# gorgonia/agogo

Measured on AMD Instinct MI355X. Metric: mcts_sims_per_sec, higher is better.
Workload: dtype f32 (Winograd F(5x5,3x3): fp32 transforms; transform-domain products as fp16x2 = each fp32 operand scaled by a power of two and split into 2 fp16 pieces (22-23 significand bits, absolute error <= 2^-38 of the tensor range), 3 fp16 MFMAs per product, fp32 accumulate)

## Files before the change

### agogo_amd/capi.py

```python
import ctypes as C
import os

import numpy as np

_HERE = os.path.dirname(os.path.abspath(__file__))
_LIB = None

NONE, BLACK, WHITE = 0, 1, 2
PASS, RESIGN = -1, -2
NO_MOVE = -32768
GAME_MNK, GAME_C4, GAME_KOMI, GAME_WQ = 0, 1, 2, 3
ENC_TWOPLANE, ENC_WQ = 0, 1
INF_NET, INF_DUMMY, INF_SCRIPT, INF_HASH, INF_UNIFORM, INF_CALLBACK = 0, 1, 2, 3, 4, 5
BN_DEGENERATE_EPS, BN_RUNNING, BN_IDENTITY = 0, 1, 2
COMPUTE_F32_MFMA, COMPUTE_BF16X3, COMPUTE_FP16X2, COMPUTE_WINO, COMPUTE_AUTO, COMPUTE_WINO_H2 = 0, 1, 2, 3, 4, 5
COMPUTE_FORCE = 0x100
PROF_CONV, PROF_HEADS, PROF_SELECT, PROF_EXPAND, PROF_MOVE, PROF_CONV_INIT = 0, 1, 2, 3, 4, 5
PROF_WINO_IN, PROF_WINO_GEMM, PROF_WINO_OUT = 6, 7, 8
DONT_PREFER_PASS, PREFER_PASS, DONT_RESIGN = 0, 1, 2
POOL_STRICT, POOL_STOP_SEARCH, POOL_GROW = 0, 1, 2


class AgzError(RuntimeError):
    pass
# ... 190 lines not shown
    sig("agz_arena_examples_dev", i32, vp, pvp, pvp, pvp, pi)
    i64, pi64 = C.c_int64, C.POINTER(C.c_int64)
    sig("agz_train_dev", i32, vp, vp, vp, vp, i32, i32, u64, pf)
    sig("agz_examples_create", i32, vp, i32, i32, i32, i32, pvp)
    sig("agz_examples_destroy", None, vp)
    sig("agz_examples_count", i32, vp, pi64)
    sig("agz_examples_clear", i32, vp)
    sig("agz_examples_append_arena", i32, vp, vp)
    sig("agz_examples_append_dev", i32, vp, vp, vp, vp, i64)
    sig("agz_examples_append_host", i32, vp, pf, pf, pf, i64)
    sig("agz_examples_get", i32, vp, pf, pf, pf, i64, pi64)
    sig("agz_examples_augment_rotate", i32, vp)
    sig("agz_examples_prepare", i32, vp, i32, i32, u64, pi)
    sig("agz_examples_tensors_dev", i32, vp, pvp, pvp, pvp, pi64, pi)
    sig("agz_examples_get_tensors", i32, vp, pf, pf, pf)
    sig("agz_examples_raw_dev", i32, vp, pvp, pvp, pvp)
    sig("agz_rotate_boards", i32, vp, pf, i32, i32, i32, pf)
    sig("agz_ctx_prof_set_stride", i32, vp, i32, i32)
    sig("agz_wino_stages", i32, vp, pf, pf, i32, i32, i32, i32, i32, pf, pf)
    sig("agz_wino_h2_tile", i32, i32, i32)
    sig("agz_net_set_wino_h2_form", i32, vp, i32)
    sig("agz_net_set_wino_h2_gemm", i32, vp, i32)
    sig("agz_net_wino_h2_last_rows", i32, vp, C.POINTER(C.c_int), C.POINTER(C.c_int))
    sig("agz_net_min_same_batch", i32, vp, i32, i32, C.POINTER(C.c_int))
    sig("agz_arena_set_prep_compact", i32, vp, i32)
    sig("agz_arena_set_split", i32, vp, i32)
    sig("agz_arena_split_steps", i32, vp, C.POINTER(C.c_int64), C.POINTER(C.c_int64), C.POINTER(C.c_int))
    sig("agz_trainer_set_dma_forward", i32, vp, i32)
    sig("agz_arena_last_prep_batch", i32, vp, C.POINTER(C.c_int), C.POINTER(C.c_int))
    sig("agz_arena_debug_counter", i32, vp, i32, C.POINTER(C.c_int64))
    sig("agz_arena_pool_capacity", i32, vp, C.POINTER(C.c_int), C.POINTER(C.c_int))
    sig("agz_wino_h2_chained", i32, i32, i32, i32)
    sig("agz_arena_random_moves", i32, vp, pi, u64)
    sig("agz_arena_set_state", i32, vp, i32, C.POINTER(State))
    sig("agz_arena_examples_labelled_dev", i32, vp, pvp)
    sig("agz_mcts_create", i32, vp, C.POINTER(GameConf), C.POINTER(MctsConf), u64, i32, pvp)
    sig("agz_mcts_destroy", None, vp)
    sig("agz_mcts_set_inferencer", i32, vp, i32, vp)
    sig("agz_mcts_set_inferencer_callback", i32, vp, INFER_FN, vp, i32)
    sig("agz_arena_set_inferencer_callback", i32, vp, i32, INFER_FN, vp, i32)
    sig("agz_arena_set_pool_policy", i32, vp, i32)
    sig("agz_mcts_set_pool_policy", i32, vp, i32)
    sig("agz_mcts_set_parallel", i32, vp, i32)
    sig("agz_mcts_set_game", i32, vp, C.POINTER(State))
    sig("agz_mcts_search", i32, vp, i32, pi)
    sig("agz_mcts_policies", i32, vp, pf, i32)
# ... 163 lines not shown
        _check(lib().agz_net_infer(self.h, _pf(x), B, _pf(pol), _pf(val)), "agz_net_infer")
        return pol, val

    def set_compute_mode(self, mode):
        _check(lib().agz_net_set_compute_mode(self.h, int(mode)), "agz_net_set_compute_mode")

    def set_latency_mode(self, on=True):
        _check(lib().agz_net_set_latency_mode(self.h, int(on)), "agz_net_set_latency_mode")

    def set_tower_queues(self, queues):
        _check(lib().agz_net_set_tower_queues(self.h, int(queues)), "agz_net_set_tower_queues")

    def set_wino_h2_form(self, form):
        _check(lib().agz_net_set_wino_h2_form(self.h, int(form)), "agz_net_set_wino_h2_form")

    def set_wino_h2_gemm(self, variant):
        _check(lib().agz_net_set_wino_h2_gemm(self.h, int(variant)), "agz_net_set_wino_h2_gemm")

    def wino_h2_last_rows(self):
        r, c = C.c_int(0), C.c_int(0)
        _check(lib().agz_net_wino_h2_last_rows(self.h, C.byref(r), C.byref(c)), "agz_net_wino_h2_last_rows")
        return r.value, c.value

    def min_same_batch(self, n, G):
        b = C.c_int(0)
        _check(lib().agz_net_min_same_batch(self.h, int(n), int(G), C.byref(b)), "agz_net_min_same_batch")
        return b.value

    def infer_dev(self, planes_ptr, B, policy_ptr, value_ptr):
        _check(lib().agz_net_infer_dev(self.h, C.c_void_p(planes_ptr), B, C.c_void_p(policy_ptr),
                                       C.c_void_p(value_ptr)), "agz_net_infer_dev")

    def flops_per_eval(self):
        return lib().agz_net_flops_per_eval(self.h)

    def save(self, path):
        _check(lib().agz_net_save(self.h, os.fsencode(path)), "agz_net_save")

    def load(self, path):
        _check(lib().agz_net_load(self.h, os.fsencode(path)), "agz_net_load")


class Trainer:

    def __init__(self, ctx, K, SharedLayers, FC, Width, Height, Features, ActionSpace, BatchSize, bn_eps=1e-5, tied=False):
        self.ctx = ctx
# ... 691 lines not shown
```

### agogo_amd/csrc/conv_wino_h2.hpp

```cpp
#pragma once

template <int TM> struct WinoT;
template <> struct WinoT<4> {
  static constexpr int AL = 6, VSHIFT = 7;
  static constexpr float BT[6][6] = {{4, 0, -5, 0, 1, 0}, {0, -4, -4, 1, 1, 0}, {0, 4, -4, -1, 1, 0}, {0, -2, -1, 2, 1, 0}, {0, 2, -1, -2, 1, 0}, {0, 4, 0, -5, 0, 1}};
  static constexpr float AT[4][6] = {{1, 1, 1, 1, 1, 0}, {0, 1, -1, 2, -2, 0}, {0, 1, 1, 4, 4, 0}, {0, 1, -1, 8, -8, 1}};
  static constexpr double G[6][3] = {{1.0 / 4, 0, 0}, {-1.0 / 6, -1.0 / 6, -1.0 / 6}, {-1.0 / 6, 1.0 / 6, -1.0 / 6}, {1.0 / 24, 1.0 / 12, 1.0 / 6}, {1.0 / 24, -1.0 / 12, 1.0 / 6}, {0, 0, 1}};
};
template <> struct WinoT<5> {
  static constexpr int AL = 7, VSHIFT = 6;
  static constexpr float BT[7][7] = {{-0.5f, 0.25f, 2.5f, -1.25f, -2, 1, 0}, {0, 0.5f, 0.25f, -2.25f, -1, 1, 0}, {0, -0.5f, 0.75f, 1.75f, -3, 1, 0},
                                     {0, 1, 1.5f, -2, -1.5f, 1, 0},          {0, -1, 2.5f, 0, -2.5f, 1, 0},       {0, 0.25f, 0, -1.25f, 0, 1, 0},
                                     {0, -0.5f, 0.25f, 2.5f, -1.25f, -2, 1}};
  static constexpr float AT[5][7] = {{1, 1, 1, 1, 1, 1, 0}, {0, 1, -1, 0.5f, -0.5f, 2, 0}, {0, 1, 1, 0.25f, 0.25f, 4, 0}, {0, 1, -1, 0.125f, -0.125f, 8, 0},
                                     {0, 1, 1, 0.0625f, 0.0625f, 16, 1}};
  static constexpr double G[7][3] = {{-2, 0, 0}, {-2.0 / 3, -2.0 / 3, -2.0 / 3}, {-2.0 / 9, 2.0 / 9, -2.0 / 9}, {16.0 / 9, 8.0 / 9, 4.0 / 9}, {16.0 / 15, -8.0 / 15, 4.0 / 15},
                                     {2.0 / 45, 4.0 / 45, 8.0 / 45}, {0, 0, 1}};
};
template <int TM> __device__ __forceinline__ void wino_btv(const float* d, float* o);
template <int TM> __device__ __forceinline__ void wino_atv(const float* m, float* o);
template <> __device__ __forceinline__ void wino_btv<4>(const float* d, float* o) { wino_bt6(d, o); }
template <> __device__ __forceinline__ void wino_atv<4>(const float* m, float* o) { wino_at4(m, o); }
template <> __device__ __forceinline__ void wino_btv<5>(const float* d, float* o) {
  o[0] = -0.5f * d[0] + 0.25f * d[1] + 2.5f * d[2] - 1.25f * d[3] - 2.f * d[4] + d[5];
// ... 25 lines not shown
  const float* w_unscale_dev;
  int fuse_prev;
  int wm_per_board;
  unsigned* amax_self;
  int in_swap;
  const _Float16* U2;
  const unsigned* amax_in;
  unsigned* amax_out;
  float* wave_max;
  float w_unscale;
  const float* t_in;
  const float* col_unscale;
  const float* t_next;
  int cform;
  const _Float16* U2c;
  const float* amax_true;
  const float* wm_prev;
  float* wm_out;
  unsigned* amax_next;
  float g1, g0;
  int gemm_variant;
  int temporal_stores;
  int live_r, live_c;
  int row_pad;
};
__device__ __forceinline__ size_t h2_row(const WinoH2Args& h, int pos, int t) {
  return (size_t)(t >> h.rsh) * h.rA + (size_t)pos * h.rB + (size_t)(t & h.rmask);
}

__device__ __forceinline__ void wino_h2_scales(unsigned amax_bits, int shift, float* s, float* inv) {
  int e = (int)((amax_bits >> 23) & 0xffu);
  if (amax_bits == 0u) { *s = 1.f; *inv = 1.f; return; }
  e = e < 30 ? 30 : (e > 230 ? 230 : e);
  *s = __uint_as_float((unsigned)(268 - shift - e) << 23);
  *inv = __uint_as_float((unsigned)(e - 14 + shift) << 23);
}

__device__ __forceinline__ unsigned wino_h2_pack(float a, float b, unsigned* lo) {
  const _Float16 ha = (_Float16)a, hb = (_Float16)b;
  const _Float16 la = (_Float16)(a - (float)ha), lb = (_Float16)(b - (float)hb);
  *lo = (unsigned)__builtin_bit_cast(unsigned short, la) | ((unsigned)__builtin_bit_cast(unsigned short, lb) << 16);
  return (unsigned)__builtin_bit_cast(unsigned short, ha) | ((unsigned)__builtin_bit_cast(unsigned short, hb) << 16);
}

template <int TM>
__global__ __launch_bounds__(256) void wino_in_h2_kernel(WinoH2Args h) {
// ... 1062 lines not shown
```

### agogo_amd/csrc/conv_wino_h2c.hpp

```cpp
#pragma once

__device__ __forceinline__ unsigned h2c_img(int row, int slot) { return maps::h2c_img(row, slot); }

template <int NK, int PFA>
__global__ __launch_bounds__(256, 2) void wino_gemm_h2c_kernel(WinoH2Args h) {
  const WinoArgs& a = h.w;
  constexpr int SA = 128 * 128, SB = 256 * 128;
  __shared__ __attribute__((aligned(16))) unsigned char lds[SA + SB];

  const int n_nt = a.Ntot >> 8;
  const int per_pos = a.n_mtiles * n_nt;
  const int nblk = h.npos * per_pos;
  const int id = blockIdx.x;
  int q = nblk >> 3, rr = nblk & 7, xcd = id & 7, slot = id >> 3;
  int tile = (xcd < rr ? xcd * (q + 1) : rr * (q + 1) + (xcd - rr) * q) + slot;
  const int pos = tile / per_pos;
  const int rem = tile - pos * per_pos;
  const int m_tile = rem / n_nt, n_tile = rem - m_tile * n_nt;

  const int tid = threadIdx.x, lane = tid & 63, wid = tid >> 6;
  const int wm = wid >> 1, wn = wid & 1;
  const unsigned st_lds = h2c_img(tid >> 3, tid & 7);
  const char* abase = reinterpret_cast<const char*>(a.V) + ((size_t)m_tile * h.npos + pos) * (size_t)NK * SA + (size_t)tid * 16;
  const char* bbase = reinterpret_cast<const char*>(h.U2c) + (((size_t)pos * NK) * n_nt + n_tile) * (size_t)SB + (size_t)tid * 16;
// ... 59 lines not shown
  float* mbase = a.Mb + ((((size_t)m_tile * h.npos + pos) * (size_t)(a.Ntot >> 6) + (size_t)n_tile * 4 + wn * 2) * 128 + (size_t)(wm * 64)) * 64 + lane;
#pragma unroll
  for (int qq = 0; qq < 2; qq++)
#pragma unroll
    for (int i = 0; i < 2; i++)
#pragma unroll
      for (int r = 0; r < 16; r++) {
        const unsigned x0 = __float_as_uint(acc[i][2 * qq][r]), x1 = __float_as_uint(acc[i][2 * qq + 1][r]);
        const auto s32 = __builtin_amdgcn_permlane32_swap(x0, x1, false, false);
        const unsigned w0 = s32[0], w1 = s32[1];
        float* d = mbase + (size_t)qq * 8192 + (size_t)(i * 32 + (r & 3) + 8 * (r >> 2)) * 64;
        d[0] = __uint_as_float(w0);
        d[4 * 64] = __uint_as_float(w1);
      }
}

typedef __attribute__((address_space(3))) void* h2c_lds_ptr_t;
template <int NK, bool NT = true>
__global__ __launch_bounds__(256, 3) void wino_gemm_h2g_kernel(WinoH2Args h) {
  const WinoArgs& a = h.w;
  constexpr int SA = 128 * 128, SB = 256 * 128;
  __shared__ __attribute__((aligned(16))) unsigned char lds[SA + SB];

  const int n_nt = a.Ntot >> 8;
  const int per_pos = a.n_mtiles * n_nt;
  const int nblk = h.npos * per_pos;
  const int id = blockIdx.x;
  int q = nblk >> 3, rr = nblk & 7, xcd = id & 7, slot = id >> 3;
  int tile = (xcd < rr ? xcd * (q + 1) : rr * (q + 1) + (xcd - rr) * q) + slot;
  const int pos = tile / per_pos;
  const int rem = tile - pos * per_pos;
  const int m_tile = rem / n_nt, n_tile = rem - m_tile * n_nt;

  const int tid = threadIdx.x, lane = tid & 63;
  const int wid = __builtin_amdgcn_readfirstlane(tid >> 6);
  const int wm = wid >> 1, wn = wid & 1;
  const __amdgpu_buffer_rsrc_t ar = h2_rsrc(a.V), br = h2_rsrc(h.U2c);
  const unsigned vo_e = maps::h2c_dma_src(lane, 0), vo_o = maps::h2c_dma_src(lane, 1);
  const unsigned a_w = maps::h2c_wave_part(wid, 128), b_w = maps::h2c_wave_part(wid, 256);
  unsigned a_so = (unsigned)(((size_t)m_tile * h.npos + pos) * (size_t)NK * SA) + a_w;
  unsigned b_so = (unsigned)((((size_t)pos * NK) * n_nt + n_tile) * (size_t)SB) + b_w;
  const unsigned b_step = (unsigned)n_nt * SB;
  unsigned char* const la = lds + a_w;
  unsigned char* const lb = lds + SA + b_w;

  f32x16 acc[2][4];
#pragma unroll
  for (int i = 0; i < 2; i++)
#pragma unroll
    for (int j = 0; j < 4; j++)
#pragma unroll
      for (int r = 0; r < 16; r++) acc[i][j][r] = 0.f;

  const int live = maps::rows_pos_live(h.live_r, h.live_c, h.tm + 2, pos);
  const bool a_on = maps::h2c_wave_row0(wid, 128) < live;
  const int ni = (maps::h2c_mfma_row0(wm, 0) < live ? 1 : 0) + (maps::h2c_mfma_row0(wm, 1) < live ? 1 : 0);
  auto k_loop = [&](auto ni_c) {
    constexpr int NI = decltype(ni_c)::value;
#pragma nounroll
    for (int it = 0; it < NK; it++) {
      if (a_on) {
#pragma unroll
        for (int j = 0; j < maps::h2c_wave_instrs(128); j++)
          __builtin_amdgcn_raw_ptr_buffer_load_lds(ar, (h2c_lds_ptr_t)(la + maps::h2c_dma_dst(0, j)), 16, (j & 1) ? vo_o : vo_e,
                                                   a_so + (maps::h2c_dma_src(0, j) - maps::h2c_dma_src(0, j & 1)), 0, 0);
      }
#pragma unroll
      for (int j = 0; j < maps::h2c_wave_instrs(256); j++)
        __builtin_amdgcn_raw_ptr_buffer_load_lds(br, (h2c_lds_ptr_t)(lb + maps::h2c_dma_dst(0, j)), 16, (j & 1) ? vo_o : vo_e,
                                                 b_so + (maps::h2c_dma_src(0, j) - maps::h2c_dma_src(0, j & 1)), 0, 0);
      a_so += SA; b_so += b_step;
      __syncthreads();
      if (NI > 0) {
#pragma unroll
        for (int ks = 0; ks < 2; ks++) {
          f16x8_t A_[2][2];
#pragma unroll
          for (int i = 0; i < NI; i++) {
            A_[i][0] = *reinterpret_cast<const f16x8_t*>(lds + maps::h2c_frag(maps::h2c_mfma_row0(wm, i), lane, 0, ks));
            A_[i][1] = *reinterpret_cast<const f16x8_t*>(lds + maps::h2c_frag(maps::h2c_mfma_row0(wm, i), lane, 1, ks));
          }
#pragma unroll
          for (int j = 0; j < 4; j++) {
            const f16x8_t b0 = *reinterpret_cast<const f16x8_t*>(lds + SA + maps::h2c_frag(wn * 128 + j * 32, lane, 0, ks));
            const f16x8_t b1 = *reinterpret_cast<const f16x8_t*>(lds + SA + maps::h2c_frag(wn * 128 + j * 32, lane, 1, ks));
#pragma unroll
            for (int i = 0; i < NI; i++) {
              acc[i][j] = __builtin_amdgcn_mfma_f32_32x32x16_f16(A_[i][1], b0, acc[i][j], 0, 0, 0);
              acc[i][j] = __builtin_amdgcn_mfma_f32_32x32x16_f16(A_[i][0], b1, acc[i][j], 0, 0, 0);
              acc[i][j] = __builtin_amdgcn_mfma_f32_32x32x16_f16(A_[i][0], b0, acc[i][j], 0, 0, 0);
            }
          }
        }
      }
      __syncthreads();
    }
  };
  if (ni == 2) k_loop(std::integral_constant<int, 2>{});
  else if (ni == 1) k_loop(std::integral_constant<int, 1>{});
  else k_loop(std::integral_constant<int, 0>{});

  float* mbase = a.Mb + maps::mc_index(m_tile, h.npos, pos, a.Ntot >> 6, n_tile * 4 + wn * 2, wm * 64, lane);
#pragma unroll
  for (int qq = 0; qq < 2; qq++)
#pragma unroll
    for (int i = 0; i < 2; i++) {
      if (i >= ni) continue;
#pragma unroll
      for (int r = 0; r < 16; r++) {
        const unsigned x0 = __float_as_uint(acc[i][2 * qq][r]), x1 = __float_as_uint(acc[i][2 * qq + 1][r]);
        const auto s32 = __builtin_amdgcn_permlane32_swap(x0, x1, false, false);
        const unsigned w0 = s32[0], w1 = s32[1];
        float* d = mbase + maps::mc_index(0, 0, 0, 0, qq, i * 32 + maps::mfma_row(r), 0);
        if (NT) {
          __builtin_nontemporal_store(__uint_as_float(w0), d);
          __builtin_nontemporal_store(__uint_as_float(w1), d + maps::mc_index(0, 0, 0, 0, 0, 4, 0));
        } else {
          d[0] = __uint_as_float(w0);
          d[maps::mc_index(0, 0, 0, 0, 0, 4, 0)] = __uint_as_float(w1);
        }
      }
    }
}


typedef unsigned h2p_rsrc_t __attribute__((ext_vector_type(4)));
__device__ __forceinline__ void h2p_dma16(h2p_rsrc_t rsrc, unsigned lds_addr, unsigned voff, unsigned soff) {
  unsigned keep;
  asm volatile("s_mov_b32 %0, m0\n\ts_mov_b32 m0, %1\n\ts_nop 0\n\tbuffer_load_dwordx4 %2, %3, %4 offen lds\n\ts_mov_b32 m0, %0"
               : "=&s"(keep) : "s"(lds_addr), "v"(voff), "s"(rsrc), "s"(soff) : "memory");
}
__device__ __forceinline__ void h2p_dma16x2(h2p_rsrc_t rsrc, unsigned lds_a, unsigned lds_b, unsigned voff_a, unsigned voff_b, unsigned soff) {
  unsigned keep;
  asm volatile("s_mov_b32 %0, m0\n\ts_mov_b32 m0, %1\n\ts_nop 0\n\tbuffer_load_dwordx4 %3, %5, %6 offen lds\n\t"
               "s_mov_b32 m0, %2\n\ts_nop 0\n\tbuffer_load_dwordx4 %4, %5, %6 offen lds\n\ts_mov_b32 m0, %0"
               : "=&s"(keep) : "s"(lds_a), "s"(lds_b), "v"(voff_a), "v"(voff_b), "s"(rsrc), "s"(soff) : "memory");
// ... 611 lines not shown
          for (int k = 0; k < 32; k++) dst[k] = src[k];
        }
      }
}

static inline bool wino_h2c_ok(int H, int W, int tm, int Kp) {
  const int tpb = ceil_div(H, tm) * ceil_div(W, tm);
  const int nk = Kp / 32;
  return Kp % 128 == 0 && 16 % tpb == 0 && (nk == 4 || nk == 8 || nk == 12 || nk == 16) &&
         (size_t)(16 / tpb) * (tm * ceil_div(H, tm) + 2) * (tm * ceil_div(W, tm) + 2) * 128 <= 80 * 1024;
}

static void wino_h2c_geometry(WinoH2Args& h) {
  WinoArgs& a = h.w;
  const int tm = h.tm == 5 ? 5 : 4;
  h.tm = tm; h.npos = (tm + 2) * (tm + 2);
  a.nty = ceil_div(a.H, tm); a.ntx = ceil_div(a.W, tm); a.TPB = a.nty * a.ntx; a.T = a.B * a.TPB;
  h.rsh = 7; h.rmask = 127; h.rA = (unsigned)h.npos * 128u; h.rB = 128u;
  a.n_mtiles = ceil_div(a.T, 128); a.n_ntiles = ceil_div(a.Ntot, 128);
  h.in_swap = 1; h.cform = 1; h.wm_per_board = 0;
}
constexpr int WINO_H2_GEMM_DEFAULT = 1;
static inline int wino_h2c_gemm_variant(const WinoH2Args& h) { return h.gemm_variant > 0 ? h.gemm_variant : WINO_H2_GEMM_DEFAULT; }
static inline bool wino_h2c_dma_ok(const WinoH2Args& h) {
  return wino_h2_rows(h.npos, (size_t)h.w.T) * h.w.C * 4 < ((size_t)1 << 31) && (size_t)h.npos * h.w.C * h.w.Ntot * 4 < ((size_t)1 << 31);
}
static inline bool wino_h2c_fits31(const WinoH2Args& h) { return wino_h2_rows(h.npos, (size_t)h.w.T) * h.w.Ntot * 4 < ((size_t)1 << 31); }
static bool wino_h2c_oip_ready(agz_ctx* ctx) {
  if (!(ctx->func_attr_state & 2u)) {
    const bool ok = hipFuncSetAttribute(reinterpret_cast<const void*>(&wino_oip_h2c_kernel<5>), hipFuncAttributeMaxDynamicSharedMemorySize, 80 * 1024) == hipSuccess &&
                    hipFuncSetAttribute(reinterpret_cast<const void*>(&wino_oip_h2c_kernel<4>), hipFuncAttributeMaxDynamicSharedMemorySize, 80 * 1024) == hipSuccess;
    if (!ok) (void)hipGetLastError();
    ctx->func_attr_state |= 2u | (ok ? 1u : 0u);
  }
  return (ctx->func_attr_state & 1u) != 0;
}
static void wino_h2c_rows(agz_ctx* ctx, WinoH2Args& h, int oi_variant, bool keep_all) {
  wino_h2c_geometry(h);
  h.live_r = h.live_c = 0;
  const int gemm = wino_h2c_gemm_variant(h) & 15;
  const maps::WinoRows g = maps::wino_rows(h.w.H, h.w.W, h.tm);
  if (keep_all || gemm != 1 || oi_variant != 4 || !wino_h2c_dma_ok(h) || !wino_h2c_fits31(h) || !maps::rows_short_ok(g) || !wino_h2c_oip_ready(ctx)) return;
  h.live_r = g.dead_y ? maps::rows_slot_live(g, maps::ROWS_R) : 0;
  h.live_c = g.dead_x ? maps::rows_slot_live(g, maps::ROWS_C) : 0;
}
static void wino_h2c_in(agz_ctx* ctx, WinoH2Args& h, hipStream_t st) {
  wino_h2c_geometry(h);
  h.fuse_prev = 0; h.amax_self = const_cast<unsigned*>(h.amax_in);
  ProfScopeOn ps(ctx, AGZ_PROF_WINO_IN, st == ctx->stream.raw());
  const size_t n_in = (size_t)h.w.T * (h.w.C / 2);
  if (h.tm == 5) hipLaunchKernelGGL(wino_in_h2_kernel<5>, dim3((unsigned)((n_in + 255) / 256)), dim3(256), 0, st, h);
  else hipLaunchKernelGGL(wino_in_h2_kernel<4>, dim3((unsigned)((n_in + 255) / 256)), dim3(256), 0, st, h);
}
static void wino_h2c_gemm(agz_ctx* ctx, WinoH2Args& h, hipStream_t st) {
  wino_h2c_geometry(h);
  ProfScopeOn ps(ctx, AGZ_PROF_WINO_GEMM, st == ctx->stream.raw());
  const dim3 g(h.npos * h.w.n_mtiles * (h.w.Ntot >> 8));
  const bool dma_ok = wino_h2c_dma_ok(h);
  const int variant_all = wino_h2c_gemm_variant(h);
  const int variant = variant_all & 15, mode = (variant_all >> 4) & 3;
  const int n_slabs = h.w.Ntot >> 7;
  if (variant == 2 && dma_ok && (h.w.C >> 5) == 8 && h.w.Ntot % 256 == 0 && ctx->num_cus / 8 >= n_slabs) {
    const dim3 gp((unsigned)(8 * ((ctx->num_cus / 8) / n_slabs) * n_slabs));
    switch (mode) {
      case 1: hipLaunchKernelGGL(wino_gemm_h2p_kernel<1>, gp, dim3(256), 0, st, h); break;
      case 2: hipLaunchKernelGGL(wino_gemm_h2p_kernel<2>, gp, dim3(256), 0, st, h); break;
      case 3: hipLaunchKernelGGL(wino_gemm_h2p_kernel<3>, gp, dim3(256), 0, st, h); break;
      default: hipLaunchKernelGGL(wino_gemm_h2p_kernel<0>, gp, dim3(256), 0, st, h); break;
    }
    return;
  }
  if (dma_ok && h.temporal_stores && (h.w.C >> 5) == 8) { hipLaunchKernelGGL((wino_gemm_h2g_kernel<8, false>), g, dim3(256), 0, st, h); return; }
  if (dma_ok) {
    switch (h.w.C >> 5) {
      case 4: hipLaunchKernelGGL((wino_gemm_h2g_kernel<4>), g, dim3(256), 0, st, h); return;
      case 8: hipLaunchKernelGGL((wino_gemm_h2g_kernel<8>), g, dim3(256), 0, st, h); return;
      case 12: hipLaunchKernelGGL((wino_gemm_h2g_kernel<12>), g, dim3(256), 0, st, h); return;
      default: hipLaunchKernelGGL((wino_gemm_h2g_kernel<16>), g, dim3(256), 0, st, h); return;
    }
  }
  switch (h.w.C >> 5) {
    case 4: hipLaunchKernelGGL((wino_gemm_h2c_kernel<4, 2>), g, dim3(256), 0, st, h); break;
    case 8: hipLaunchKernelGGL((wino_gemm_h2c_kernel<8, 2>), g, dim3(256), 0, st, h); break;
    case 12: hipLaunchKernelGGL((wino_gemm_h2c_kernel<12, 2>), g, dim3(256), 0, st, h); break;
    default: hipLaunchKernelGGL((wino_gemm_h2c_kernel<16, 2>), g, dim3(256), 0, st, h); break;
  }
}
static void wino_h2c_oi(agz_ctx* ctx, WinoH2Args& h, bool last, hipStream_t st, int variant = 4) {
  wino_h2c_geometry(h);
  ProfScopeOn ps(ctx, AGZ_PROF_WINO_OUT, st == ctx->stream.raw());
  const WinoArgs& a = h.w;
  const dim3 g((unsigned)ceil_div(a.T, 16), (unsigned)(a.C >> 5));
  const size_t shm = last ? 0 : (size_t)(16 / a.TPB) * a.H * a.W * 32 * sizeof(float);
  const bool fits31 = wino_h2c_fits31(h);
  if (variant == 4 && !last && fits31 && wino_h2c_oip_ready(ctx)) {
    const size_t shp = (size_t)(16 / a.TPB) * (h.tm * a.nty + 2) * (h.tm * a.ntx + 2) * 32 * sizeof(float);
    const int items = ceil_div(a.T, 16) * (a.C >> 5);
    const dim3 gp((unsigned)std::min(items, 2 * ctx->num_cus));
    if (h.tm == 5 && h.temporal_stores) {
      (void)hipFuncSetAttribute(reinterpret_cast<const void*>(&wino_oip_h2c_kernel<5, false>), hipFuncAttributeMaxDynamicSharedMemorySize, 80 * 1024);
      hipLaunchKernelGGL((wino_oip_h2c_kernel<5, false>), gp, dim3(256), shp, st, h);
      return;
    }
    if (h.tm == 5) hipLaunchKernelGGL((wino_oip_h2c_kernel<5>), gp, dim3(256), shp, st, h);
    else hipLaunchKernelGGL((wino_oip_h2c_kernel<4>), gp, dim3(256), shp, st, h);
    return;
  }
  if (h.tm == 5) {
    if (last) hipLaunchKernelGGL((wino_oi_h2c_kernel<5, true>), g, dim3(256), shm, st, h);
// ... 7 lines not shown
```

### agogo_amd/csrc/gemm_maps.hpp

```cpp
#pragma once
#include <cstddef>
#if defined(__HIPCC__)
#define AGZ_MAPS_HD __host__ __device__
#else
#define AGZ_MAPS_HD
#endif

namespace agz {
namespace maps {

AGZ_MAPS_HD constexpr unsigned h2c_img(int row, int unit) { return (unsigned)(row * 128 + ((unit ^ ((row >> 1) & 7)) << 4)); }

AGZ_MAPS_HD constexpr unsigned h2c_dma_src(int lane, int j) {
  return (unsigned)(j * 1024 + (lane >> 3) * 128 + (((lane & 7) ^ ((4 * j + (lane >> 4)) & 7)) << 4));
}
AGZ_MAPS_HD constexpr unsigned h2c_dma_dst(int lane, int j) { return (unsigned)(j * 1024 + lane * 16); }
AGZ_MAPS_HD constexpr unsigned h2c_wave_part(int wid, int stage_rows) { return (unsigned)(wid * (stage_rows / 4) * 128); }
AGZ_MAPS_HD constexpr int h2c_wave_instrs(int stage_rows) { return stage_rows / 4 / 8; }

AGZ_MAPS_HD constexpr unsigned h2c_frag(int row0, int lane, int piece, int ks) {
  return (unsigned)((row0 + (lane & 31)) * 128 + (((piece * 4 + 2 * ks + (lane >> 5)) ^ ((lane >> 1) & 7)) << 4));
}

AGZ_MAPS_HD constexpr int mfma_row(int r) { return (r & 3) + 8 * (r >> 2); }
// ... 19 lines not shown
}
AGZ_MAPS_HD constexpr int rows_local(int cls, int nty, int ntx, int ty, int tx) {
  return cls == ROWS_R ? (ty < nty - 1 ? ty * ntx + tx : -1) : (cls == ROWS_C ? (tx < ntx - 1 ? ty * (ntx - 1) + tx : -1) : ty * ntx + tx);
}
AGZ_MAPS_HD constexpr int rows_row(int cls, int nty, int ntx, int bs, int ty, int tx) {
  return rows_local(cls, nty, ntx, ty, tx) < 0 ? -1 : bs * rows_per_board(cls, nty, ntx) + rows_local(cls, nty, ntx, ty, tx);
}
AGZ_MAPS_HD constexpr int rows_slot_live(const WinoRows& g, int cls) { return g.bpt * rows_per_board(cls, g.nty, g.ntx); }
AGZ_MAPS_HD constexpr bool rows_live_ok(int live) { return live == 32 || live == 64 || live == 96; }
AGZ_MAPS_HD constexpr bool rows_short_ok(const WinoRows& g) {
  return 128 % g.TPB == 0 && (g.dead_y || g.dead_x) && (!g.dead_y || rows_live_ok(rows_slot_live(g, ROWS_R))) &&
         (!g.dead_x || rows_live_ok(rows_slot_live(g, ROWS_C)));
}
AGZ_MAPS_HD constexpr int rows_pos_live(int live_r, int live_c, int AL, int pos) {
  return pos / AL == AL - 1 ? (live_r ? live_r : 128) : ((live_c && pos % AL == AL - 1) ? live_c : 128);
}
AGZ_MAPS_HD constexpr int rows_stored_per_board(const WinoRows& g) {
  int n = 0;
  for (int xi = 0; xi < g.AL; xi++)
    for (int nu = 0; nu < g.AL; nu++) n += rows_per_board(rows_class(g.dead_y, g.dead_x, g.AL, xi, nu), g.nty, g.ntx);
  return n;
}

constexpr int H2P_D = 10, H2P_R = 16, H2P_NK = 8;
AGZ_MAPS_HD constexpr unsigned h2p_v_base(int pos, int hm, int npos) {
  return (unsigned)(((hm >> 1) * npos + pos) * (H2P_NK * 16384) + (hm & 1) * 8192);
}
AGZ_MAPS_HD constexpr int h2p_slot(int par, int kk) { return (par * H2P_NK + kk) % H2P_R; }
AGZ_MAPS_HD constexpr int h2p_slot_next(int par, int kk) { return (par * H2P_NK + kk + 1) % H2P_R; }
AGZ_MAPS_HD constexpr int h2p_slot_ahead(int par, int kk) { return (par * H2P_NK + kk + H2P_D) % H2P_R; }
AGZ_MAPS_HD constexpr int h2p_kk_ahead(int kk) { return (kk + H2P_D) % H2P_NK; }
AGZ_MAPS_HD constexpr int h2p_tiles_ahead(int kk) { return (kk + H2P_D) / H2P_NK; }
AGZ_MAPS_HD constexpr int h2p_wait_steady() { return 4 + (H2P_D - 2) * 6; }
AGZ_MAPS_HD constexpr int h2p_wait_early() { return (H2P_D - 2) * 2; }
AGZ_MAPS_HD constexpr bool h2p_early(int t) { return t < 2; }
struct H2pTeam { int team, slab, nteams; bool idle; };
AGZ_MAPS_HD constexpr H2pTeam h2p_team(int block, int grid, int n_slabs) {
  const int xcd = block & 7, slot = block >> 3, tpx = (grid >> 3) / n_slabs;
  return H2pTeam{xcd * tpx + (tpx ? slot / n_slabs : 0), tpx ? slot % n_slabs : 0, 8 * tpx, slot >= tpx * n_slabs};
}
AGZ_MAPS_HD constexpr int h2p_u0(int team, int nteams, int U2) { return 2 * (int)((long)team * U2 / nteams); }

}
}
```

### agogo_amd/csrc/net.hip

```cpp
#include "net.hpp"
#include "gemm_maps.hpp"

#include <cmath>
#include <cstdio>
#include <cstring>
#include <type_traits>

typedef float f32x16 __attribute__((ext_vector_type(16)));
typedef float f32x4 __attribute__((ext_vector_type(4)));

namespace agz {

struct ConvArgs {
  const float* x;
  const float* w;
  const void* ep;
  float* y;
  int M, HW, W, Wp, HpWp;
  int Cin_p, Cout_p, Ntot;
  int n_mtiles, n_ntiles;
  int raw;
  int splits;
  int per;
  float* ws;
// ... 1077 lines not shown
  return AGZ_OK;
}

void agz_net::wino_h2c_block(int l, int B, int b0, int ci, const H2Tower& t, hipStream_t st, float* cur, float* nxt) {
  const size_t wmb = (size_t)t.tpb * (Kp >> 5);
  const bool last = l + 1 == conf.SharedLayers;
  float* d_wave_max = reinterpret_cast<float*>(d_amax + (size_t)(conf.SharedLayers + 1) * B);
  WinoH2Args hh{};
  WinoArgs& wa = hh.w;
  wa.x = cur + (size_t)b0 * Hp * Wp * Kp; wa.y = nxt + (size_t)b0 * Hp * Wp * Kp;
  wa.V = d_wV + (size_t)ci * t.v_elems; wa.Mb = d_wM + (size_t)ci * t.m_elems; wa.ep = d_ep_h2[l];
  wa.B = std::min(t.chunk, B - b0); wa.H = H; wa.W = W; wa.Hp = Hp; wa.Wp = Wp; wa.C = Kp; wa.Cout_p = Kp; wa.Ntot = 2 * Kp;
  hh.U2c = d_u2c_dual[l]; hh.w_unscale = 1.f; hh.tm = wino_tm;
  hh.amax_in = d_amax + (size_t)l * B + b0;
  hh.amax_next = last ? nullptr : d_amax + (size_t)(l + 1) * B + b0;
  hh.amax_true = l == 0 ? reinterpret_cast<const float*>(d_amax + b0) : nullptr;
  hh.wm_prev = d_wave_max + ((size_t)((l + 1) & 1) * B + b0) * wmb;
  hh.wm_out = d_wave_max + ((size_t)(l & 1) * B + b0) * wmb;
  hh.g1 = wino_g1[l]; hh.g0 = wino_g0[l];
  {
    static const int gemm_env = [] {
      const char* e = getenv("AGZ_WINO_H2_GEMM");
      const int v = e ? atoi(e) : 0;
      if (v == 0 || (((v & 63) == 1 || (v & 63) == 2) && (v >> 6) <= 3)) return v;
      fprintf(stderr, "libagz: AGZ_WINO_H2_GEMM=%s ignored (want 1 or 2, optionally + 64 and / or + 128)\n", e);
      return 0;
    }();
    const int gv = wino_gemm > 0 ? wino_gemm : gemm_env;
    hh.gemm_variant = gv & 63; hh.temporal_stores = (gv >> 6) & 1;
    agz::wino_h2c_rows(ctx, hh, t.form_want == 1 ? 1 : 4, ((gv >> 7) & 1) != 0);
    wino_live_r = hh.live_r; wino_live_c = hh.live_c;
  }
  if (l == 0) agz::wino_h2c_in(ctx, hh, st);
  agz::wino_h2c_gemm(ctx, hh, st);
  agz::wino_h2c_oi(ctx, hh, last, st, t.form_want == 1 ? 1 : 4);
}

void agz_net::heads_spread_range(agz::HeadArgs h, bool nb4, int B, int b0, int nb, hipStream_t st) {
  h.x += (size_t)b0 * Hp * Wp * Kp;
  h.feat = d_hs + (size_t)b0 * 3 * HW; h.cols = d_hs + (size_t)B * 3 * HW + (size_t)b0 * (conf.ActionSpace + conf.FC);
  h.policy += (size_t)b0 * conf.ActionSpace; h.value += b0;
  hipLaunchKernelGGL(heads_feat_kernel, dim3(ceil_div(HW, 4), nb), dim3(256), 0, st, h);
  if (nb4)
    hipLaunchKernelGGL(heads_fc_nb_kernel<4>, dim3(ceil_div(conf.ActionSpace + conf.FC, 64), ceil_div(nb, 4)), dim3(1024), 0, st, h, nb);
  else
    hipLaunchKernelGGL(heads_fc_kernel, dim3(ceil_div(conf.ActionSpace + conf.FC, 64), nb), dim3(1024), 0, st, h);
  hipLaunchKernelGGL(heads_out_kernel, dim3(nb), dim3(256), 0, st, h);
}

bool agz_net::half_ok(int B) const {
  if (!committed || B < 2 || B > max_batch || (B & 1) || (B / 2) % 4 != 0 || cfg != 0 || conf.SharedLayers <= 0) return false;
  if (min_same_batch(B / 2, B) != B / 2) return false;
  const FwdPlan plan = fwd_plan(B);
  int mode = compute_mode;
  if (mode == AGZ_COMPUTE_AUTO) mode = !d_u2_dual.empty() ? AGZ_COMPUTE_WINO_H2 : AGZ_COMPUTE_BF16X3;
  if (!plan.split_ok || plan.latency || mode != AGZ_COMPUTE_WINO_H2 || !plan.heads_spread || !plan.heads_nb) return false;
  if ((int)d_u2_dual.size() != conf.SharedLayers || !d_ep_init_h2) return false;
// ... 615 lines not shown
  return form_env != 0 && agz::wino_h2c_ok(H, W, agz::wino_h2_pick_tm(H, W), Kp) ? 1 : 0;
}

int agz_net_set_wino_h2_form(agz_net* n, int form) {
  AGZ_REQUIRE(n, AGZ_E_INVALID, "agz_net_set_wino_h2_form: null net");
  AGZ_REQUIRE(form >= -1 && form <= 2, AGZ_E_INVALID, "agz_net_set_wino_h2_form: form %d (want -1, 0 or 1)", form);
  n->wino_form = form;
  return AGZ_OK;
}

int agz_net_min_same_batch(agz_net* n, int k, int G, int* batch) {
  AGZ_REQUIRE(n && batch && k >= 1 && G >= k, AGZ_E_INVALID, "agz_net_min_same_batch: bad argument");
  AGZ_REQUIRE(n->committed, AGZ_E_STATE, "agz_net_min_same_batch: commit the net first");
  *batch = n->min_same_batch(k, G);
  return AGZ_OK;
}

int agz_net_wino_h2_last_rows(agz_net* n, int* live_r, int* live_c) {
  AGZ_REQUIRE(n && live_r && live_c, AGZ_E_INVALID, "agz_net_wino_h2_last_rows: null argument");
  *live_r = n->wino_live_r; *live_c = n->wino_live_c;
  return AGZ_OK;
}

int agz_net_set_wino_h2_gemm(agz_net* n, int variant) {
  AGZ_REQUIRE(n, AGZ_E_INVALID, "agz_net_set_wino_h2_gemm: null net");
  AGZ_REQUIRE(((variant & 63) <= 2 && (variant >> 6) <= 3) || ((variant & 15) == 2 && (variant >> 4) <= 3), AGZ_E_INVALID, "agz_net_set_wino_h2_gemm: variant %d (want 0, 1, 2, + 64, + 128, or 2 + 16 * mode)", variant);
  n->wino_gemm = variant;
  return AGZ_OK;
}

int agz_wino_stages(agz_ctx* ctx, const float* x, const float* w, int B, int H, int W, int C, int N, float* V, float* M) {
  AGZ_REQUIRE(ctx && x && w && V && M, AGZ_E_INVALID, "agz_wino_stages: NULL argument");
  AGZ_REQUIRE(B >= 1 && H >= 1 && W >= 1 && C >= 16 && C % 16 == 0 && N >= 1, AGZ_E_INVALID, "agz_wino_stages: bad shape");
  AGZ_HIP_TRY(hipSetDevice(ctx->device));
  const int Hp = H + 2, Wp = W + 2;
  std::vector<float> xp((size_t)B * Hp * Wp * C, 0.f);
  for (int b = 0; b < B; b++) for (int h = 0; h < H; h++)
    memcpy(&xp[(((size_t)b * Hp + h + 1) * Wp + 1) * C], &x[((size_t)b * H + h) * W * C], (size_t)W * C * sizeof(float));
  std::vector<unsigned short> u3;
  agz::wino_build_u3(u3, N, C, [&](int n, int ci, int tap) -> double { return (double)w[((size_t)n * C + ci) * 9 + tap]; });
  agz::WinoArgs a{};
  a.B = B; a.H = H; a.W = W; a.Hp = Hp; a.Wp = Wp; a.C = C; a.Cout_p = N; a.Ntot = N;
  const size_t T = (size_t)B * agz::ceil_div(H, 4) * agz::ceil_div(W, 4);
  AGZ_REQUIRE((size_t)36 * T * C * 4 < ((size_t)1 << 32), AGZ_E_UNSUPPORTED, "agz_wino_stages: V above 4 GiB");
  float *dx = nullptr, *dV = nullptr, *dM = nullptr;
  unsigned short* dU = nullptr;
  int rc = AGZ_OK;
  if (hipMalloc(&dx, xp.size() * 4) != hipSuccess || hipMalloc(&dV, (size_t)36 * T * C * 4) != hipSuccess ||
      hipMalloc(&dM, (size_t)36 * T * N * 4) != hipSuccess || hipMalloc(&dU, u3.size() * 2) != hipSuccess) {
// ... 120 lines not shown
```

### agogo_amd/csrc/net.hpp

```cpp
#pragma once
#include <string>
#include <vector>

#include "common.hpp"

namespace agz {
struct Param {
  std::string name;
  std::vector<float> v;
  std::vector<int> ref_shape;
  int kind;
};
struct BNStats { std::vector<float> mean, var; };
int conv3x3_raw(agz_ctx* ctx, const float* x, const float* w, float* y, int B, int H, int W, int Cin_p, int Cout_p);
int conv3x3_raw_x3(agz_ctx* ctx, const float* x, const unsigned short* w3, float* y, int B, int H, int W, int Cin_p, int Cout_p);
int split_w3(agz_ctx* ctx, const float* w, unsigned short* w3, int N, int Cin_p);
inline size_t w3_elems(int N, int Cin_p) { return (size_t)9 * 3 * N * Cin_p; }
struct WinoRawScratch {
  float* V = nullptr; float* M = nullptr; void* U2 = nullptr; unsigned* words = nullptr;
  size_t v_cap = 0, m_cap = 0, u_cap = 0; int b_cap = 0;
  void* w2 = nullptr; unsigned* h2_words = nullptr;
  size_t w2_cap = 0; int h2_b_cap = 0, h2_flip = 0;
};
int conv3x3_raw_h2(agz_ctx* ctx, const float* x, const float* w, float* y, int B, int H, int W, int Cin_p, int Cout_p, WinoRawScratch* sc,
// ... 20 lines not shown

  int H = 0, W = 0, HW = 0, Hp = 0, Wp = 0;
  int Kp = 0;
  int Fp = 32;
  int cfg = 0;

  float* d_w_init = nullptr;
  float* d_w_init_t = nullptr;
  float* d_ep_init = nullptr;
  unsigned short* d_w3_init = nullptr;
  std::vector<float*> d_w_dual;
  std::vector<float*> d_ep_dual;
  std::vector<unsigned short*> d_w3_dual;
  std::vector<_Float16*> d_w2_dual;
  std::vector<float> w_unscale;
  std::vector<unsigned short*> d_u3_dual;
  std::vector<_Float16*> d_u2_dual;
  std::vector<float> u_unscale;
  std::vector<float*> d_u2_tin;
  std::vector<float*> d_u2_colun;
  std::vector<_Float16*> d_u2c_dual;
  std::vector<float> wino_g1, wino_g0;
  int wino_gemm = 0;
  int wino_live_r = 0, wino_live_c = 0;
  int wino_form = -1;
  void free_u2c() { for (auto& p : d_u2c_dual) if (p) hipFree(p); d_u2c_dual.clear(); wino_g1.clear(); wino_g0.clear(); }
  int build_wino_h2_weights();
  int wino_tm = 4;
  size_t wino_v_cap = 0;
  float* d_wV = nullptr;
  float* d_wM = nullptr;
  int wino_chunk_cap = 0;
  int build_wino_weights();
  unsigned* d_amax = nullptr;
  size_t amax_cap = 0;
  int compute_mode = AGZ_COMPUTE_F32_MFMA;
  bool compute_force = false;
  float* d_head_conv = nullptr;
  float* d_head_bn = nullptr;
  float* d_Wp = nullptr;
  float* d_bp = nullptr;
  float* d_W1 = nullptr;
  float* d_b1 = nullptr;
  float* d_W2 = nullptr;
  float* d_b2 = nullptr;

// ... 39 lines not shown
```

### include/agz_debug.h

```cpp
#ifndef AGZ_DEBUG_H
#define AGZ_DEBUG_H

#include "agz.h"

#ifdef __cplusplus
extern "C" {
#endif

#define AGZ_PROF_CONV 0
#define AGZ_PROF_HEADS 1
#define AGZ_PROF_SELECT 2
#define AGZ_PROF_EXPAND 3
#define AGZ_PROF_MOVE 4
#define AGZ_PROF_CONV_INIT 5
#define AGZ_PROF_WINO_IN 6
#define AGZ_PROF_WINO_GEMM 7
#define AGZ_PROF_WINO_OUT 8
#define AGZ_PROF_NCLASS 9
int agz_ctx_prof_enable(agz_ctx* ctx, int enable);
int agz_ctx_prof_read(agz_ctx* ctx, int klass, int64_t* launches, double* total_ms);
int agz_ctx_prof_set_stride(agz_ctx* ctx, int klass, int stride);

int agz_wino_stages(agz_ctx* ctx, const float* x, const float* w, int B, int H, int W, int C, int N, float* V, float* M);

int agz_wino_h2_tile(int H, int W);

int agz_wino_h2_chained(int H, int W, int K);

int agz_net_set_wino_h2_form(agz_net* net, int form);

int agz_net_set_wino_h2_gemm(agz_net* net, int variant);

int agz_net_wino_h2_last_rows(agz_net* net, int* live_r, int* live_c);

int agz_arena_set_prep_compact(agz_arena* arena, int on);
int agz_arena_last_prep_batch(agz_arena* arena, int* boards, int* roots);

int agz_arena_set_split(agz_arena* arena, int mode);
int agz_arena_split_steps(agz_arena* arena, int64_t* split, int64_t* joined, int* last_split);

int agz_trainer_set_dma_forward(agz_trainer* t, int on);

int agz_net_min_same_batch(agz_net* net, int n, int G, int* batch);

#define AGZ_CNT_PATHMAX 15
int agz_arena_debug_counter(agz_arena* arena, int which, int64_t* value);

int agz_arena_pool_capacity(agz_arena* arena, int* nodes_per_pool, int* grows);

int agz_comm_debug_fail_slice(agz_comm* comm, int k);

int agz_comm_debug_fail_layer(agz_comm* comm, int layer);

#ifdef __cplusplus
}
#endif
#endif
// ... 1 lines not shown
```

Baseline: 44440.

## Compact Winograd fp16x2 GEMM grid to live row blocks per transform position

The Winograd GEMM kernel now decodes its workgroup from a compact work list. For transform positions whose rows are only partly live (the last row or column of the tile), it packs 32-row blocks from several m-tiles into one workgroup, so fewer workgroups are launched for padded rows. Each wave's A and M addressing is recomputed per 32-row block, and reciprocal-multiply division keeps the decode cheap. The list is on by default through a new constant, and an env or variant bit can turn it off. A debug query reports the launched grid size.

Result: no change. 44020 (-0.9%).

```diff
diff --git a/agogo_amd/capi.py b/agogo_amd/capi.py
--- a/agogo_amd/capi.py
+++ b/agogo_amd/capi.py
@@ -236,6 +236,7 @@
     sig("agz_net_set_wino_h2_form", i32, vp, i32)
     sig("agz_net_set_wino_h2_gemm", i32, vp, i32)
     sig("agz_net_wino_h2_last_rows", i32, vp, C.POINTER(C.c_int), C.POINTER(C.c_int))
+    sig("agz_net_wino_h2_last_gemm_grid", i32, vp, C.POINTER(C.c_int))
     sig("agz_net_min_same_batch", i32, vp, i32, i32, C.POINTER(C.c_int))
     sig("agz_arena_set_prep_compact", i32, vp, i32)
     sig("agz_arena_set_split", i32, vp, i32)
@@ -445,6 +446,11 @@
         _check(lib().agz_net_wino_h2_last_rows(self.h, C.byref(r), C.byref(c)), "agz_net_wino_h2_last_rows")
         return r.value, c.value
 
+    def wino_h2_last_gemm_grid(self):
+        n = C.c_int(0)
+        _check(lib().agz_net_wino_h2_last_gemm_grid(self.h, C.byref(n)), "agz_net_wino_h2_last_gemm_grid")
+        return n.value
+
     def min_same_batch(self, n, G):
         b = C.c_int(0)
         _check(lib().agz_net_min_same_batch(self.h, int(n), int(G), C.byref(b)), "agz_net_min_same_batch")
diff --git a/agogo_amd/csrc/conv_wino_h2.hpp b/agogo_amd/csrc/conv_wino_h2.hpp
--- a/agogo_amd/csrc/conv_wino_h2.hpp
+++ b/agogo_amd/csrc/conv_wino_h2.hpp
@@ -71,6 +71,8 @@
   int gemm_variant;
   int temporal_stores;
   int live_r, live_c;
+  int block_list;
+  maps::GemmList gl;
   int row_pad;
 };
 __device__ __forceinline__ size_t h2_row(const WinoH2Args& h, int pos, int t) {
diff --git a/agogo_amd/csrc/conv_wino_h2c.hpp b/agogo_amd/csrc/conv_wino_h2c.hpp
--- a/agogo_amd/csrc/conv_wino_h2c.hpp
+++ b/agogo_amd/csrc/conv_wino_h2c.hpp
@@ -105,23 +105,21 @@
   constexpr int SA = 128 * 128, SB = 256 * 128;
   __shared__ __attribute__((aligned(16))) unsigned char lds[SA + SB];
 
-  const int n_nt = a.Ntot >> 8;
-  const int per_pos = a.n_mtiles * n_nt;
-  const int nblk = h.npos * per_pos;
-  const int id = blockIdx.x;
-  int q = nblk >> 3, rr = nblk & 7, xcd = id & 7, slot = id >> 3;
-  int tile = (xcd < rr ? xcd * (q + 1) : rr * (q + 1) + (xcd - rr) * q) + slot;
-  const int pos = tile / per_pos;
-  const int rem = tile - pos * per_pos;
-  const int m_tile = rem / n_nt, n_tile = rem - m_tile * n_nt;
+  const int n_nt = h.gl.n_nt;
+  const maps::GemmUnit un = maps::gemm_decode(h.gl, maps::gemm_xcd_tile((int)blockIdx.x, maps::gemm_grid(h.gl)));
+  const int pos = un.pos, n_tile = un.n_tile;
 
   const int tid = threadIdx.x, lane = tid & 63;
   const int wid = __builtin_amdgcn_readfirstlane(tid >> 6);
   const int wm = wid >> 1, wn = wid & 1;
+  const int live = maps::rows_pos_live(h.live_r, h.live_c, h.tm + 2, pos);
+  const maps::GemmBlock blk_a = maps::gemm_block(h.gl.n_mtiles, un, live, wid);
+  const maps::GemmBlock blk_m[2] = {maps::gemm_block(h.gl.n_mtiles, un, live, 2 * wm),
+                                    maps::gemm_block(h.gl.n_mtiles, un, live, 2 * wm + 1)};
   const __amdgpu_buffer_rsrc_t ar = h2_rsrc(a.V), br = h2_rsrc(h.U2c);
   const unsigned vo_e = maps::h2c_dma_src(lane, 0), vo_o = maps::h2c_dma_src(lane, 1);
   const unsigned a_w = maps::h2c_wave_part(wid, 128), b_w = maps::h2c_wave_part(wid, 256);
-  unsigned a_so = (unsigned)(((size_t)m_tile * h.npos + pos) * (size_t)NK * SA) + a_w;
+  unsigned a_so = maps::gemm_a_base(blk_a.slot, h.npos, pos, NK, blk_a.blk);
   unsigned b_so = (unsigned)((((size_t)pos * NK) * n_nt + n_tile) * (size_t)SB) + b_w;
   const unsigned b_step = (unsigned)n_nt * SB;
   unsigned char* const la = lds + a_w;
@@ -135,9 +133,8 @@
 #pragma unroll
       for (int r = 0; r < 16; r++) acc[i][j][r] = 0.f;
 
-  const int live = maps::rows_pos_live(h.live_r, h.live_c, h.tm + 2, pos);
-  const bool a_on = maps::h2c_wave_row0(wid, 128) < live;
-  const int ni = (maps::h2c_mfma_row0(wm, 0) < live ? 1 : 0) + (maps::h2c_mfma_row0(wm, 1) < live ? 1 : 0);
+  const bool a_on = blk_a.on;
+  const int ni = (blk_m[0].on ? 1 : 0) + (blk_m[1].on ? 1 : 0);
   auto k_loop = [&](auto ni_c) {
     constexpr int NI = decltype(ni_c)::value;
 #pragma nounroll
@@ -183,7 +180,8 @@
   else if (ni == 1) k_loop(std::integral_constant<int, 1>{});
   else k_loop(std::integral_constant<int, 0>{});
 
-  float* mbase = a.Mb + maps::mc_index(m_tile, h.npos, pos, a.Ntot >> 6, n_tile * 4 + wn * 2, wm * 64, lane);
+  float* const mbase[2] = {a.Mb + maps::mc_index(blk_m[0].slot, h.npos, pos, a.Ntot >> 6, n_tile * 4 + wn * 2, blk_m[0].blk * 32, lane),
+                           a.Mb + maps::mc_index(blk_m[1].slot, h.npos, pos, a.Ntot >> 6, n_tile * 4 + wn * 2, blk_m[1].blk * 32, lane)};
 #pragma unroll
   for (int qq = 0; qq < 2; qq++)
 #pragma unroll
@@ -194,7 +192,7 @@
         const unsigned x0 = __float_as_uint(acc[i][2 * qq][r]), x1 = __float_as_uint(acc[i][2 * qq + 1][r]);
         const auto s32 = __builtin_amdgcn_permlane32_swap(x0, x1, false, false);
         const unsigned w0 = s32[0], w1 = s32[1];
-        float* d = mbase + maps::mc_index(0, 0, 0, 0, qq, i * 32 + maps::mfma_row(r), 0);
+        float* d = mbase[i] + maps::mc_index(0, 0, 0, 0, qq, maps::mfma_row(r), 0);
         if (NT) {
           __builtin_nontemporal_store(__uint_as_float(w0), d);
           __builtin_nontemporal_store(__uint_as_float(w1), d + maps::mc_index(0, 0, 0, 0, 0, 4, 0));
@@ -852,6 +850,7 @@
 }
 constexpr int WINO_H2_GEMM_DEFAULT = 1;
 static inline int wino_h2c_gemm_variant(const WinoH2Args& h) { return h.gemm_variant > 0 ? h.gemm_variant : WINO_H2_GEMM_DEFAULT; }
+constexpr int WINO_H2_GEMM_BLOCKS_DEFAULT = 1;
 static inline bool wino_h2c_dma_ok(const WinoH2Args& h) {
   return wino_h2_rows(h.npos, (size_t)h.w.T) * h.w.C * 4 < ((size_t)1 << 31) && (size_t)h.npos * h.w.C * h.w.Ntot * 4 < ((size_t)1 << 31);
 }
@@ -882,10 +881,12 @@
   if (h.tm == 5) hipLaunchKernelGGL(wino_in_h2_kernel<5>, dim3((unsigned)((n_in + 255) / 256)), dim3(256), 0, st, h);
   else hipLaunchKernelGGL(wino_in_h2_kernel<4>, dim3((unsigned)((n_in + 255) / 256)), dim3(256), 0, st, h);
 }
-static void wino_h2c_gemm(agz_ctx* ctx, WinoH2Args& h, hipStream_t st) {
+static unsigned wino_h2c_gemm(agz_ctx* ctx, WinoH2Args& h, hipStream_t st) {
   wino_h2c_geometry(h);
   ProfScopeOn ps(ctx, AGZ_PROF_WINO_GEMM, st == ctx->stream.raw());
   const dim3 g(h.npos * h.w.n_mtiles * (h.w.Ntot >> 8));
+  h.gl = maps::gemm_list(h.w.n_mtiles, h.w.Ntot >> 8, h.tm + 2, h.block_list ? h.live_r : 0, h.block_list ? h.live_c : 0);
+  const dim3 gd((unsigned)maps::gemm_grid(h.gl));
   const bool dma_ok = wino_h2c_dma_ok(h);
   const int variant_all = wino_h2c_gemm_variant(h);
   const int variant = variant_all & 15, mode = (variant_all >> 4) & 3;
@@ -898,15 +899,15 @@
       case 3: hipLaunchKernelGGL(wino_gemm_h2p_kernel<3>, gp, dim3(256), 0, st, h); break;
       default: hipLaunchKernelGGL(wino_gemm_h2p_kernel<0>, gp, dim3(256), 0, st, h); break;
     }
-    return;
-  }
-  if (dma_ok && h.temporal_stores && (h.w.C >> 5) == 8) { hipLaunchKernelGGL((wino_gemm_h2g_kernel<8, false>), g, dim3(256), 0, st, h); return; }
+    return gp.x;
+  }
+  if (dma_ok && h.temporal_stores && (h.w.C >> 5) == 8) { hipLaunchKernelGGL((wino_gemm_h2g_kernel<8, false>), gd, dim3(256), 0, st, h); return gd.x; }
   if (dma_ok) {
     switch (h.w.C >> 5) {
-      case 4: hipLaunchKernelGGL((wino_gemm_h2g_kernel<4>), g, dim3(256), 0, st, h); return;
-      case 8: hipLaunchKernelGGL((wino_gemm_h2g_kernel<8>), g, dim3(256), 0, st, h); return;
-      case 12: hipLaunchKernelGGL((wino_gemm_h2g_kernel<12>), g, dim3(256), 0, st, h); return;
-      default: hipLaunchKernelGGL((wino_gemm_h2g_kernel<16>), g, dim3(256), 0, st, h); return;
+      case 4: hipLaunchKernelGGL((wino_gemm_h2g_kernel<4>), gd, dim3(256), 0, st, h); return gd.x;
+      case 8: hipLaunchKernelGGL((wino_gemm_h2g_kernel<8>), gd, dim3(256), 0, st, h); return gd.x;
+      case 12: hipLaunchKernelGGL((wino_gemm_h2g_kernel<12>), gd, dim3(256), 0, st, h); return gd.x;
+      default: hipLaunchKernelGGL((wino_gemm_h2g_kernel<16>), gd, dim3(256), 0, st, h); return gd.x;
     }
   }
   switch (h.w.C >> 5) {
@@ -915,6 +916,7 @@
     case 12: hipLaunchKernelGGL((wino_gemm_h2c_kernel<12, 2>), g, dim3(256), 0, st, h); break;
     default: hipLaunchKernelGGL((wino_gemm_h2c_kernel<16, 2>), g, dim3(256), 0, st, h); break;
   }
+  return g.x;
 }
 static void wino_h2c_oi(agz_ctx* ctx, WinoH2Args& h, bool last, hipStream_t st, int variant = 4) {
   wino_h2c_geometry(h);
diff --git a/agogo_amd/csrc/gemm_maps.hpp b/agogo_amd/csrc/gemm_maps.hpp
--- a/agogo_amd/csrc/gemm_maps.hpp
+++ b/agogo_amd/csrc/gemm_maps.hpp
@@ -65,6 +65,45 @@
   return n;
 }
 
+AGZ_MAPS_HD constexpr unsigned gemm_inv(int d) { return (unsigned)((((unsigned long long)1 << 31) + (unsigned)d - 1) / (unsigned)d); }
+AGZ_MAPS_HD constexpr int gemm_div(int x, unsigned inv) { return (int)(((unsigned long long)(unsigned)x * inv) >> 31); }
+struct GemmList {
+  int n_nt, n_mtiles, AL, fc, lb1, lb2, upp1, upp2, end0, end1, units;
+  unsigned inv_nt, inv_upp0, inv_upp1, inv_upp2, inv_fc, inv_lb1, inv_lb2;
+};
+AGZ_MAPS_HD constexpr int gemm_units_per_pos(int n_mtiles, int lb) { return (n_mtiles * lb + 3) / 4; }
+AGZ_MAPS_HD constexpr GemmList gemm_list(int n_mtiles, int n_nt, int AL, int list_r, int list_c) {
+  const int fc = list_c ? AL - 1 : AL, lb1 = list_c ? list_c / 32 : 4, lb2 = list_r ? list_r / 32 : 4;
+  const int upp1 = gemm_units_per_pos(n_mtiles, lb1), upp2 = gemm_units_per_pos(n_mtiles, lb2);
+  const int end0 = (AL - 1) * fc * n_mtiles, end1 = end0 + (AL - 1) * (AL - fc) * upp1;
+  return GemmList{n_nt, n_mtiles, AL, fc, lb1, lb2, upp1, upp2, end0, end1, end1 + AL * upp2,
+                  gemm_inv(n_nt), gemm_inv(n_mtiles), gemm_inv(upp1), gemm_inv(upp2), gemm_inv(fc), gemm_inv(lb1), gemm_inv(lb2)};
+}
+AGZ_MAPS_HD constexpr int gemm_grid(const GemmList& g) { return g.units * g.n_nt; }
+AGZ_MAPS_HD constexpr int gemm_xcd_tile(int id, int nblk) {
+  const int q = nblk >> 3, rr = nblk & 7, xcd = id & 7, slot = id >> 3;
+  return (xcd < rr ? xcd * (q + 1) : rr * (q + 1) + (xcd - rr) * q) + slot;
+}
+struct GemmUnit { int pos, unit, n_tile, lb; unsigned inv_lb; };
+AGZ_MAPS_HD constexpr GemmUnit gemm_decode(const GemmList& g, int tile) {
+  const int u = gemm_div(tile, g.inv_nt), n_tile = tile - u * g.n_nt;
+  const int reg = u < g.end0 ? 0 : (u < g.end1 ? 1 : 2);
+  const int off = reg == 0 ? 0 : (reg == 1 ? g.end0 : g.end1), upp = reg == 0 ? g.n_mtiles : (reg == 1 ? g.upp1 : g.upp2);
+  const int p = gemm_div(u - off, reg == 0 ? g.inv_upp0 : (reg == 1 ? g.inv_upp1 : g.inv_upp2)), unit = (u - off) - p * upp;
+  const int pr = reg == 0 ? gemm_div(p, g.inv_fc) : (reg == 1 ? p : 0), w = reg == 0 ? g.fc : (reg == 1 ? 1 : g.AL);
+  const int base = reg == 0 ? 0 : (reg == 1 ? g.AL - 1 : (g.AL - 1) * g.AL);
+  return GemmUnit{base + pr * g.AL + (p - pr * w), unit, n_tile, reg == 0 ? 4 : (reg == 1 ? g.lb1 : g.lb2),
+                  reg == 0 ? gemm_inv(4) : (reg == 1 ? g.inv_lb1 : g.inv_lb2)};
+}
+struct GemmBlock { int slot, blk; bool on; };
+AGZ_MAPS_HD constexpr GemmBlock gemm_block(int n_mtiles, const GemmUnit& un, int live, int j) {
+  const int k = 4 * un.unit + j, slot = gemm_div(k, un.inv_lb), blk = k - slot * un.lb;
+  return GemmBlock{slot, blk, slot < n_mtiles && 32 * blk < live};
+}
+AGZ_MAPS_HD constexpr unsigned gemm_a_base(int slot, int npos, int pos, int nk, int blk) {
+  return (unsigned)(((size_t)slot * npos + pos) * (size_t)nk * 16384 + (size_t)blk * 4096);
+}
+
 constexpr int H2P_D = 10, H2P_R = 16, H2P_NK = 8;
 AGZ_MAPS_HD constexpr unsigned h2p_v_base(int pos, int hm, int npos) {
   return (unsigned)(((hm >> 1) * npos + pos) * (H2P_NK * 16384) + (hm & 1) * 8192);
diff --git a/agogo_amd/csrc/net.hip b/agogo_amd/csrc/net.hip
--- a/agogo_amd/csrc/net.hip
+++ b/agogo_amd/csrc/net.hip
@@ -1123,17 +1123,18 @@
     static const int gemm_env = [] {
       const char* e = getenv("AGZ_WINO_H2_GEMM");
       const int v = e ? atoi(e) : 0;
-      if (v == 0 || (((v & 63) == 1 || (v & 63) == 2) && (v >> 6) <= 3)) return v;
-      fprintf(stderr, "libagz: AGZ_WINO_H2_GEMM=%s ignored (want 1 or 2, optionally + 64 and / or + 128)\n", e);
+      if (v == 0 || (((v & 63) == 1 || (v & 63) == 2) && (v >> 6) <= 15 && (v & 768) != 768)) return v;
+      fprintf(stderr, "libagz: AGZ_WINO_H2_GEMM=%s ignored (want 1 or 2, optionally + 64, + 128 and one of + 256, + 512)\n", e);
       return 0;
     }();
     const int gv = wino_gemm > 0 ? wino_gemm : gemm_env;
     hh.gemm_variant = gv & 63; hh.temporal_stores = (gv >> 6) & 1;
+    hh.block_list = (gv & 512) ? 1 : ((gv & 256) ? 0 : agz::WINO_H2_GEMM_BLOCKS_DEFAULT);
     agz::wino_h2c_rows(ctx, hh, t.form_want == 1 ? 1 : 4, ((gv >> 7) & 1) != 0);
     wino_live_r = hh.live_r; wino_live_c = hh.live_c;
   }
   if (l == 0) agz::wino_h2c_in(ctx, hh, st);
-  agz::wino_h2c_gemm(ctx, hh, st);
+  wino_gemm_grid = (int)agz::wino_h2c_gemm(ctx, hh, st);
   agz::wino_h2c_oi(ctx, hh, last, st, t.form_want == 1 ? 1 : 4);
 }
 
@@ -1795,9 +1796,16 @@
   return AGZ_OK;
 }
 
+int agz_net_wino_h2_last_gemm_grid(agz_net* n, int* workgroups) {
+  AGZ_REQUIRE(n && workgroups, AGZ_E_INVALID, "agz_net_wino_h2_last_gemm_grid: null argument");
+  *workgroups = n->wino_gemm_grid;
+  return AGZ_OK;
+}
+
 int agz_net_set_wino_h2_gemm(agz_net* n, int variant) {
   AGZ_REQUIRE(n, AGZ_E_INVALID, "agz_net_set_wino_h2_gemm: null net");
-  AGZ_REQUIRE(((variant & 63) <= 2 && (variant >> 6) <= 3) || ((variant & 15) == 2 && (variant >> 4) <= 3), AGZ_E_INVALID, "agz_net_set_wino_h2_gemm: variant %d (want 0, 1, 2, + 64, + 128, or 2 + 16 * mode)", variant);
+  AGZ_REQUIRE(((variant & 63) <= 2 && (variant >> 6) <= 15 && (variant & 768) != 768) || ((variant & 15) == 2 && (variant >> 4) <= 3), AGZ_E_INVALID,
+              "agz_net_set_wino_h2_gemm: variant %d (want 0, 1, 2, + 64, + 128, + 256 or + 512, or 2 + 16 * mode)", variant);
   n->wino_gemm = variant;
   return AGZ_OK;
 }
diff --git a/agogo_amd/csrc/net.hpp b/agogo_amd/csrc/net.hpp
--- a/agogo_amd/csrc/net.hpp
+++ b/agogo_amd/csrc/net.hpp
@@ -66,6 +66,7 @@
   std::vector<_Float16*> d_u2c_dual;
   std::vector<float> wino_g1, wino_g0;
   int wino_gemm = 0;
+  int wino_gemm_grid = 0;
   int wino_live_r = 0, wino_live_c = 0;
   int wino_form = -1;
   void free_u2c() { for (auto& p : d_u2c_dual) if (p) hipFree(p); d_u2c_dual.clear(); wino_g1.clear(); wino_g0.clear(); }
diff --git a/include/agz_debug.h b/include/agz_debug.h
--- a/include/agz_debug.h
+++ b/include/agz_debug.h
@@ -33,6 +33,8 @@
 
 int agz_net_wino_h2_last_rows(agz_net* net, int* live_r, int* live_c);
 
+int agz_net_wino_h2_last_gemm_grid(agz_net* net, int* workgroups);
+
 int agz_arena_set_prep_compact(agz_arena* arena, int on);
 int agz_arena_last_prep_batch(agz_arena* arena, int* boards, int* roots);
 
```
